# bgmanuel99/Super-Resolution-Images-for-3D-Printing-Defect-Detection

Measured on AMD Instinct MI355X. Metric: 4x-SR MPix/s on 512x512 LR batch, higher is better.
Workload: dtype bf16

## Files before the change

__graft_entry__.py:

```python
import os
import subprocess
import sys

ROOT = os.path.dirname(os.path.abspath(__file__))
PKG = os.path.join(ROOT, "super-resolution-images-for-3d-printing-defect-detection_amd")
for p in (ROOT, PKG):
    if p not in sys.path:
        sys.path.insert(0, p)


def build():
    jobs = str(min(4, os.cpu_count() or 1))
    subprocess.run(["make", "-C", os.path.join(PKG, "csrc"), "-j", jobs], check=True)
    subprocess.run([sys.executable, os.path.join(ROOT, "tools", "check_prefetch_hazards.py")], check=True)
    import sr355
    from sr355 import _lib
    _lib.load()
    import SRModels.loading_methods
    import oracle


def smoke():
    import numpy as np
    import torch
    assert torch.cuda.is_available(), "smoke() needs a GPU"
    from oracle import models as OM
    from oracle import ops as OO
    from sr355 import Context
    from sr355.synth import make_pairs
    from sr355.weights import bf16_rounded, init_weights
    from SRModels.deep_learning_models.ESRGAN_model import ESRGAN

    ctx = Context.get(0)
    lr, hr = make_pairs(1, 40, 36, 4, seed=7)
    for dtype, tol in (("f32", 1e-4), ("bf16", 2e-2)):
        m = ESRGAN(compute_dtype=dtype)
        m.setup_model(scale_factor=4, growth_channels=32, num_rrdb_blocks=2)
        w = init_weights(m.generator.layer_shapes(), seed=3000)
        if dtype == "bf16":
            w = bf16_rounded(w)
        m.set_weights(w)
        sr, metrics = m.super_resolve_image(lr[0], patch_size_lr=24, stride=12)
        ref = OM.esrgan_super_resolve(lr[0], w, 4, 24, 12, num_rrdb=2, dtype=np.float64)
        err = float(np.abs(sr - ref).max())
        assert sr.shape == (160, 144, 3) and err <= tol, (dtype, err)
        p_gpu = float(ctx.psnr(ctx.to_device(hr), ctx.to_device(sr[None]))[0])
        p_ref = float(OO.psnr(hr, ref[None].astype(np.float32))[0])
        assert abs(p_gpu - p_ref) <= 0.01, (p_gpu, p_ref)
        print(f"smoke[{dtype}]: max|gpu-oracle|={err:.2e}  PSNR(gpu,HR)={p_gpu:.4f} dB  PSNR(oracle,HR)={p_ref:.4f} dB  "
              f"time_sec={metrics['time_sec']:.4f}")
    print("smoke OK")


if __name__ == "__main__":
    build()
    if len(sys.argv) > 1 and sys.argv[1] == "smoke":
        smoke()
```

super-resolution-images-for-3d-printing-defect-detection_amd/csrc/attention.hip:

```cpp
#include "attn_f32.h"
#include "common.h"

#include <cstdlib>

namespace {

struct AttnParams {
    const char* qkv; int64_t cs; int qoff, koff, voff;
    char* o; int64_t o_cs; int o_coff;
    int N;
    const float* knorm;
};

__global__ void __launch_bounds__(256, 2) attn_f32_kernel(AttnParams p) {
    __shared__ __attribute__((aligned(16))) char vt[32 * ATTN_VT_PITCH];
    const int b = blockIdx.y;
    const float* base = reinterpret_cast<const float*>(p.qkv) + (int64_t)b * p.N * p.cs;
    const AttnF32Args a{base + p.qoff, base + p.koff, base + p.voff, p.cs, p.cs, p.cs,
                        reinterpret_cast<float*>(p.o) + (int64_t)b * p.N * p.o_cs + p.o_coff, p.o_cs, nullptr, p.N};
    attn_f32_body<false>(a, blockIdx.x * 128, vt);
}

constexpr int KT2 = 128;
constexpr int PITCH2 = KT2 * 2 + 8;

__global__ void __launch_bounds__(64) attn_knorm_kernel(const bf16_t* qkv, int64_t cs, int koff, int N, int ngroups, float* out) {
    const int g = blockIdx.x % ngroups, b = blockIdx.x / ngroups, lane = threadIdx.x;
    const bf16_t* base = qkv + (int64_t)b * N * cs + koff;
    float m = 0.f;
#pragma unroll
    for (int t = 0; t < 2; ++t) {
        const int key = g * 128 + t * 64 + lane;
        if (key < N) {
            const bf16x8 k = *reinterpret_cast<const bf16x8*>(base + (int64_t)key * cs);
            float n2 = 0.f;
#pragma unroll
            for (int e = 0; e < 8; ++e) n2 += (float)k[e] * (float)k[e];
            m = fmaxf(m, n2);
        }
    }
#pragma unroll
    for (int o = 32; o > 0; o >>= 1) m = fmaxf(m, __shfl_xor(m, o));
    if (lane == 0) out[(int64_t)b * ngroups + g] = sqrtf(m);
}

template <int QB>
__global__ void __launch_bounds__(256, 3) attn_bf16_kernel(AttnParams p) {
    __shared__ __attribute__((aligned(16))) char vt[32 * PITCH2];
    const int tid = threadIdx.x, lane = tid & 63, wave = tid >> 6, r = lane & 31, h = lane >> 5;
    const int N = p.N;
    constexpr int QW = 64 * QB * 2;
    const int nqt = (N + QW - 1) / QW;
    const int b = blockIdx.x / nqt, qt = blockIdx.x - b * nqt;
    const bf16_t* base = reinterpret_cast<const bf16_t*>(p.qkv) + (int64_t)b * N * p.cs;
    const int cs = (int)p.cs;
    int qi[QB];
    bf16x8 qb[QB];
#pragma unroll
    for (int j = 0; j < QB; ++j) {
        qi[j] = qt * QW + wave * (32 * QB) + j * 32 + r;
        const int qc = qi[j] < N ? qi[j] : N - 1;
        bf16x8 z = {};
        qb[j] = z;
        if (h == 0) qb[j] = *reinterpret_cast<const bf16x8*>(base + (int64_t)qc * cs + p.qoff);
    }
    float qn2 = 0.f;
#pragma unroll
    for (int j = 0; j < QB; ++j) {
        float n2 = 0.f;
#pragma unroll
        for (int e = 0; e < 8; ++e) n2 += (float)qb[j][e] * (float)qb[j][e];
        qn2 = fmaxf(qn2, n2);
    }
#pragma unroll
    for (int o = 32; o > 0; o >>= 1) qn2 = fmaxf(qn2, __shfl_xor(qn2, o));
    const float qmaxv = sqrtf(qn2) * 1.0009765625f;
    const int* knorm_bits = reinterpret_cast<const int*>(p.knorm) + (int64_t)b * ((N + KT2 - 1) / KT2);
    f32x16 oacc[QB];
    bf16x8 sel = {};
    {
        const int m = lane & 15, kg = lane >> 4;
        const bf16_t one = (bf16_t)1.f;
        if ((m == 0 && (kg & 1) == 0) || (m == 1 && (kg & 1) == 1)) sel = bf16x8{one, one, one, one, one, one, one, one};
    }
    f32x4 lacc[QB];
    float m_run[QB];
#pragma unroll
    for (int j = 0; j < QB; ++j) {
        m_run[j] = 0.f; lacc[j] = f32x4{0.f, 0.f, 0.f, 0.f};
#pragma unroll
        for (int e = 0; e < 16; ++e) oacc[j][e] = 0.f;
    }

    const int kp = tid >> 2, oct = tid & 3;
    bf16x8 kneg = {};
    kneg[0] = (bf16_t)-1.f; kneg[1] = (bf16_t)-1.f; kneg[2] = (bf16_t)-1.f;
    auto load_k = [&](int kb) {
        int l;
        asm volatile("v_mbcnt_lo_u32_b32 %0, -1, 0\n\tv_mbcnt_hi_u32_b32 %0, -1, %0" : "=v"(l));
        bf16x8 kf = kneg;
        const int key = kb + (l & 31);
        if (l < 32) kf = *reinterpret_cast<const bf16x8*>(base + (int64_t)(key < N ? key : N - 1) * cs + p.koff);
        return kf;
    };
    bf16x8 knext = load_k(0);
    f32x16 zero16;
#pragma unroll
    for (int e = 0; e < 16; ++e) zero16[e] = 0.f;
    struct { } false_c; struct { int x; } true_c{0};
    auto hmax = [](float v) {
        const unsigned u = __builtin_bit_cast(unsigned, v);
        const auto sw = __builtin_amdgcn_permlane32_swap(u, u, false, false);
        return fmaxf(__builtin_bit_cast(float, (unsigned)sw[0]), __builtin_bit_cast(float, (unsigned)sw[1]));
    };
    auto tile = [&](const bf16x8 kf, const int sub, const int kb, auto ragged_tag, const bool first) {
        constexpr bool RAGGED = sizeof(ragged_tag) > 1;
        f32x16 s[QB];
        float mx[QB];
#pragma unroll
        for (int j = 0; j < QB; ++j) {
            s[j] = __builtin_amdgcn_mfma_f32_32x32x16_bf16(kf, qb[j], zero16, 0, 0, 0);
            if constexpr (RAGGED) {
#pragma unroll
                for (int i = 0; i < 16; ++i)
                    if (kb + (i & 3) + 8 * (i >> 2) + 4 * h >= N) s[j][i] = -INFINITY;
            }
            float m = fmaxf(fmaxf(s[j][0], s[j][1]), s[j][2]);
#pragma unroll
            for (int i = 3; i + 1 < 16; i += 2) m = fmaxf(fmaxf(m, s[j][i]), s[j][i + 1]);
            m = fmaxf(m, s[j][15]);
            mx[j] = hmax(m);
        }
        bool grew = first;
#pragma unroll
        for (int j = 0; j < QB; ++j) grew = grew || mx[j] > 0.f;
        if (__any(grew)) {
#pragma unroll
            for (int j = 0; j < QB; ++j) {
                const float delta = first ? mx[j] : fmaxf(mx[j], 0.f);
                const float alpha = first ? 1.f : __builtin_amdgcn_exp2f(-delta);
                lacc[j][0] *= alpha;
                lacc[j][1] *= __shfl(alpha, (lane + 16) & 63);
#pragma unroll
                for (int e = 0; e < 16; ++e) oacc[j][e] *= alpha;
#pragma unroll
                for (int i = 0; i < 16; ++i) s[j][i] -= delta;
                m_run[j] += delta;
                if (h == 1) {
                    const bf16_t m1 = (bf16_t)m_run[j];
                    const float r1 = m_run[j] - (float)m1;
                    const bf16_t m2 = (bf16_t)r1;
                    qb[j][0] = m1; qb[j][1] = m2; qb[j][2] = (bf16_t)(r1 - (float)m2);
                }
            }
        }
#pragma unroll
        for (int j = 0; j < QB; ++j) {
#pragma unroll
            for (int i = 0; i < 16; ++i) s[j][i] = __builtin_amdgcn_exp2f(s[j][i]);
        }
#pragma unroll
        for (int ks = 0; ks < 2; ++ks) {
            const char* vrow = vt + r * PITCH2 + (sub * 32 + 16 * ks + 4 * h) * 2;
            const bf16x4 va = *reinterpret_cast<const bf16x4*>(vrow);
            const bf16x4 vb = *reinterpret_cast<const bf16x4*>(vrow + 16);
            const bf16x8 vf = {va[0], va[1], va[2], va[3], vb[0], vb[1], vb[2], vb[3]};
#pragma unroll
            for (int j = 0; j < QB; ++j) {
                bf16x8 pf;
#pragma unroll
                for (int e = 0; e < 8; ++e) pf[e] = (bf16_t)s[j][8 * ks + e];
                oacc[j] = __builtin_amdgcn_mfma_f32_32x32x16_bf16(vf, pf, oacc[j], 0, 0, 0);
                lacc[j] = __builtin_amdgcn_mfma_f32_16x16x32_bf16(sel, pf, lacc[j], 0, 0, 0);
            }
        }
    };

    constexpr float GROW_OK = 40.f;
    auto tile_fast = [&](const bf16x8 kf, const int sub, const bool guard) -> bool {
        f32x16 s[QB];
#pragma unroll
        for (int j = 0; j < QB; ++j) s[j] = __builtin_amdgcn_mfma_f32_32x32x16_bf16(kf, qb[j], zero16, 0, 0, 0);
        if (guard) {
            bool risky = false;
#pragma unroll
            for (int j = 0; j < QB; ++j) {
                float m = fmaxf(fmaxf(s[j][0], s[j][1]), s[j][2]);
#pragma unroll
                for (int i = 3; i + 1 < 16; i += 2) m = fmaxf(fmaxf(m, s[j][i]), s[j][i + 1]);
                m = fmaxf(m, s[j][15]);
                risky = risky || m > GROW_OK;
            }
            if (__any(risky)) return false;
        }
#pragma unroll
        for (int j = 0; j < QB; ++j) {
#pragma unroll
            for (int i = 0; i < 16; ++i) s[j][i] = __builtin_amdgcn_exp2f(s[j][i]);
        }
#pragma unroll
        for (int ks = 0; ks < 2; ++ks) {
            const char* vrow = vt + r * PITCH2 + (sub * 32 + 16 * ks + 4 * h) * 2;
            const bf16x4 va = *reinterpret_cast<const bf16x4*>(vrow);
            const bf16x4 vb = *reinterpret_cast<const bf16x4*>(vrow + 16);
            const bf16x8 vf = {va[0], va[1], va[2], va[3], vb[0], vb[1], vb[2], vb[3]};
#pragma unroll
            for (int j = 0; j < QB; ++j) {
                bf16x8 pf;
#pragma unroll
                for (int e = 0; e < 8; ++e) pf[e] = (bf16_t)s[j][8 * ks + e];
                oacc[j] = __builtin_amdgcn_mfma_f32_32x32x16_bf16(vf, pf, oacc[j], 0, 0, 0);
                lacc[j] = __builtin_amdgcn_mfma_f32_16x16x32_bf16(sel, pf, lacc[j], 0, 0, 0);
            }
        }
        return true;
    };
    auto thresh_of_wave = [&]() -> int {
        float m = m_run[0];
#pragma unroll
        for (int j = 1; j < QB; ++j) m = fminf(m, m_run[j]);
#pragma unroll
        for (int o = 32; o > 0; o >>= 1) m = fminf(m, __shfl_xor(m, o));
        const float lim = GROW_OK + m;
        const float th = !(lim >= 0.f) ? -1.f : (qmaxv > 0.f ? lim / qmaxv * 0.9990234375f : INFINITY);
        return __builtin_amdgcn_readfirstlane(__builtin_bit_cast(int, th));
    };
    int thresh_bits = __builtin_amdgcn_readfirstlane(__builtin_bit_cast(int, -1.f));
    auto stage_v = [&](const int k0) {
        __syncthreads();
#pragma unroll
        for (int part = 0; part < KT2 / 128; ++part) {
            const int ka = k0 + part * 128 + 2 * kp, kbb = ka + 1;
            if (ka - 2 * kp >= N) break;
            const bf16x8 va = *reinterpret_cast<const bf16x8*>(base + (int64_t)(ka < N ? ka : N - 1) * cs + p.voff + oct * 8);
            const bf16x8 vb = *reinterpret_cast<const bf16x8*>(base + (int64_t)(kbb < N ? kbb : N - 1) * cs + p.voff + oct * 8);
#pragma unroll
            for (int e = 0; e < 8; ++e) {
                typedef bf16_t bf16x2 __attribute__((ext_vector_type(2)));
                bf16x2 pr = {va[e], vb[e]};
                *reinterpret_cast<bf16x2*>(vt + (oct * 8 + e) * PITCH2 + (part * 64 + kp) * 4) = pr;
            }
        }
        __syncthreads();
    };
    auto slow_tiles = [&](const int k0, const int sub0, bf16x8 kf) {
        for (int sub = sub0; sub < KT2 / 32; ++sub) {
            const int kb = k0 + sub * 32;
            if (kb >= N) break;
            if (sub != sub0) { kf = knext; knext = load_k(kb + 32); }
            if (kb + 32 <= N) tile(kf, sub, kb, false_c, kb == 0);
            else tile(kf, sub, kb, true_c, kb == 0);
        }
    };

    for (int k0 = 0; k0 < N; k0 += KT2) {
        stage_v(k0);
        int sub = 0;
        bf16x8 kf = knext;
        const bool full = k0 != 0 && k0 + KT2 <= N;
        if (full) {
            const bool guard = !(knorm_bits[k0 / KT2] <= thresh_bits);
#pragma unroll
            for (; sub < KT2 / 32; ++sub) {
                kf = knext;
                knext = load_k(k0 + sub * 32 + 32);
                if (!tile_fast(kf, sub, guard)) break;
            }
        } else {
            knext = load_k(k0 + 32);
        }
        if (sub < KT2 / 32) {
            slow_tiles(k0, sub, kf);
            thresh_bits = thresh_of_wave();
        }
    }
#pragma unroll
    for (int j = 0; j < QB; ++j) {
        const float l0 = __shfl(lacc[j][0], r & 15), l1 = __shfl(lacc[j][1], r & 15);
        const float inv = 1.f / ((r >> 4) ? l1 : l0);
        if (qi[j] < N) {
            bf16_t* op = reinterpret_cast<bf16_t*>(p.o) + ((int64_t)b * N + qi[j]) * p.o_cs + p.o_coff;
#pragma unroll
            for (int g = 0; g < 4; ++g) {
                bf16x4 t = {(bf16_t)(oacc[j][4 * g] * inv), (bf16_t)(oacc[j][4 * g + 1] * inv), (bf16_t)(oacc[j][4 * g + 2] * inv),
                            (bf16_t)(oacc[j][4 * g + 3] * inv)};
                *reinterpret_cast<bf16x4*>(op + 8 * g + 4 * h) = t;
            }
        }
    }
}

}

int attention_launch(sr_ctx* ctx, int dtype, const void* qkv, int64_t cs, int qoff, int koff, int voff, int B, int N,
                     void* o, int64_t o_cs, int o_coff, hipStream_t st) {
    if (B <= 0 || N <= 0) return ctx->fail(SR_ERR_INVALID, "attention: empty tensor");
    const int esz = dtype_size(dtype);
    if ((cs * esz) % 16 || (qoff * esz) % 16 || (koff * esz) % 16 || (voff * esz) % 16 || (o_cs * esz) % 16 || (o_coff * esz) % 16)
        return ctx->fail(SR_ERR_INVALID, "attention: views must be 16-byte aligned");
    AttnParams p{static_cast<const char*>(qkv), cs, qoff, koff, voff, static_cast<char*>(o), o_cs, o_coff, N, nullptr};
    dim3 grid((unsigned)((N + 127) / 128), (unsigned)B);
    if (dtype != SR_DTYPE_BF16 && dtype != SR_DTYPE_F32) return ctx->fail(SR_ERR_INVALID, "attention: dtype must be f32 or bf16");
    const int rec = ctx->prof_open(dtype == SR_DTYPE_BF16 ? "attn<bf16>" : "attn<f32>", 2.0 * B * (double)N * N * 40.0,
                                   (double)B * N * 80.0 * esz, st);
    if (dtype == SR_DTYPE_BF16) {
        constexpr int QBr = 2;
        const int64_t nwg = (int64_t)B * ((N + 128 * QBr - 1) / (128 * QBr));
        const int ngroups = (N + KT2 - 1) / KT2;
        if (nwg >= (1ll << 31) || (int64_t)B * ngroups >= (1ll << 31)) { ctx->prof_close(rec, st); return ctx->fail(SR_ERR_INVALID, "attention: too many workgroups for one launch"); }
        float* kn = static_cast<float*>(ctx->arena(ctx->attn_kn, sizeof(float) * (size_t)B * ngroups, st));
        if (!kn) { ctx->prof_close(rec, st); return SR_ERR_OOM; }
        p.knorm = kn;
        hipLaunchKernelGGL(attn_knorm_kernel, dim3((unsigned)((int64_t)B * ngroups)), dim3(64), 0, st, reinterpret_cast<const bf16_t*>(qkv) + 0, cs, koff, N, ngroups, kn);
        hipLaunchKernelGGL(attn_bf16_kernel<QBr>, dim3((unsigned)nwg), dim3(256), 0, st, p);
    }
    else hipLaunchKernelGGL(attn_f32_kernel, grid, dim3(256), 0, st, p);
    ctx->prof_close(rec, st);
    SR_HIP(ctx, hipGetLastError());
    return SR_OK;
}
```

Before: 110.4.

## Add batched fast path for consecutive skippable-free attention key tiles with asm prefetch

Adds a fast loop in the bf16 attention kernel that uses a wave ballot over precomputed key norms to find a run of consecutive KV blocks where the unguarded fast tile path is safe. Those blocks are then processed without bounds checks or per-tile guards, using inline-asm double-buffered K loads that issue the next tile's global load while the current tile's MFMAs run. The change also specializes V staging for whole tiles to drop clamping. It relies on hand-written waitcnt and exec manipulation, which is why a prefetch hazard checker is added to the build. It also risks register-allocation and correctness issues.

```diff
diff --git a/__graft_entry__.py b/__graft_entry__.py
--- a/__graft_entry__.py
+++ b/__graft_entry__.py
@@ -13,6 +13,8 @@
     jobs = str(min(4, os.cpu_count() or 1))
     subprocess.run(["make", "-C", os.path.join(PKG, "csrc"), "-j", jobs], check=True)
     subprocess.run([sys.executable, os.path.join(ROOT, "tools", "check_prefetch_hazards.py")], check=True)
+    subprocess.run([sys.executable, os.path.join(ROOT, "tools", "check_prefetch_hazards.py"), "--source", os.path.join(PKG, "csrc", "attention.hip"),
+                    "--match", "attn_bf16_kernel", "--allow-scratch"], check=True)
     import sr355
     from sr355 import _lib
     _lib.load()
diff --git a/super-resolution-images-for-3d-printing-defect-detection_amd/csrc/attention.hip b/super-resolution-images-for-3d-printing-defect-detection_amd/csrc/attention.hip
--- a/super-resolution-images-for-3d-printing-defect-detection_amd/csrc/attention.hip
+++ b/super-resolution-images-for-3d-printing-defect-detection_amd/csrc/attention.hip
@@ -226,14 +226,15 @@
         return __builtin_amdgcn_readfirstlane(__builtin_bit_cast(int, th));
     };
     int thresh_bits = __builtin_amdgcn_readfirstlane(__builtin_bit_cast(int, -1.f));
-    auto stage_v = [&](const int k0) {
+    auto stage_v = [&](const int k0, auto whole_tag) {
+        constexpr bool WHOLE = sizeof(whole_tag) > 1;
         __syncthreads();
 #pragma unroll
         for (int part = 0; part < KT2 / 128; ++part) {
             const int ka = k0 + part * 128 + 2 * kp, kbb = ka + 1;
-            if (ka - 2 * kp >= N) break;
-            const bf16x8 va = *reinterpret_cast<const bf16x8*>(base + (int64_t)(ka < N ? ka : N - 1) * cs + p.voff + oct * 8);
-            const bf16x8 vb = *reinterpret_cast<const bf16x8*>(base + (int64_t)(kbb < N ? kbb : N - 1) * cs + p.voff + oct * 8);
+            if (!WHOLE && ka - 2 * kp >= N) break;
+            const bf16x8 va = *reinterpret_cast<const bf16x8*>(base + (int64_t)(WHOLE || ka < N ? ka : N - 1) * cs + p.voff + oct * 8);
+            const bf16x8 vb = *reinterpret_cast<const bf16x8*>(base + (int64_t)(WHOLE || kbb < N ? kbb : N - 1) * cs + p.voff + oct * 8);
 #pragma unroll
             for (int e = 0; e < 8; ++e) {
                 typedef bf16_t bf16x2 __attribute__((ext_vector_type(2)));
@@ -253,25 +254,65 @@
         }
     };
 
-    for (int k0 = 0; k0 < N; k0 += KT2) {
-        stage_v(k0);
-        int sub = 0;
-        bf16x8 kf = knext;
-        const bool full = k0 != 0 && k0 + KT2 <= N;
-        if (full) {
-            const bool guard = !(knorm_bits[k0 / KT2] <= thresh_bits);
-#pragma unroll
-            for (; sub < KT2 / 32; ++sub) {
-                kf = knext;
-                knext = load_k(k0 + sub * 32 + 32);
-                if (!tile_fast(kf, sub, guard)) break;
-            }
-        } else {
-            knext = load_k(k0 + 32);
-        }
-        if (sub < KT2 / 32) {
-            slow_tiles(k0, sub, kf);
-            thresh_bits = thresh_of_wave();
+    const unsigned kvoff = (unsigned)r * (unsigned)cs * 2u;
+    auto fetch_k = [&](bf16x8& use, bf16x8& next, const char* tile_base) {
+        asm volatile("s_waitcnt vmcnt(0)\n\ts_mov_b32 exec_hi, 0\n\tglobal_load_dwordx4 %1, %2, %3\n\ts_mov_b32 exec_hi, -1"
+                     : "+v"(use), "+v"(next) : "v"(kvoff), "s"(tile_base) : "memory");
+    };
+    const int nfast = N % KT2 == 0 ? N / KT2 : (N - 32) / KT2;
+    auto fast_run = [&](const int g) -> int {
+        if (g >= nfast) return 0;
+        int l;
+        asm volatile("v_mbcnt_lo_u32_b32 %0, -1, 0\n\tv_mbcnt_hi_u32_b32 %0, -1, %0" : "=v"(l));
+        const int gi = g + l;
+        const bool ok = gi < nfast && knorm_bits[gi < nfast ? gi : nfast - 1] <= thresh_bits;
+        const unsigned long long fails = ~__ballot(ok);
+        return fails ? __builtin_ctzll(fails) : 64;
+    };
+    const char* const kimg = reinterpret_cast<const char*>(base + p.koff);
+    const int64_t tile_bytes = (int64_t)32 * cs * 2;
+
+    for (int k0 = 0; k0 < N;) {
+        {
+            stage_v(k0, false_c);
+            int sub = 0;
+            bf16x8 kf = knext;
+            const bool full = k0 != 0 && k0 + KT2 <= N;
+            if (full) {
+                const bool guard = !(knorm_bits[k0 / KT2] <= thresh_bits);
+#pragma unroll
+                for (; sub < KT2 / 32; ++sub) {
+                    kf = knext;
+                    knext = load_k(k0 + sub * 32 + 32);
+                    if (!tile_fast(kf, sub, guard)) break;
+                }
+            } else {
+                knext = load_k(k0 + 32);
+            }
+            if (sub < KT2 / 32) {
+                slow_tiles(k0, sub, kf);
+                thresh_bits = thresh_of_wave();
+            }
+            k0 += KT2;
+        }
+        int run = fast_run(k0 / KT2);
+        if (run > 0) {
+            bf16x8 ka = knext, kb = kneg;
+            const char* kt = kimg + (int64_t)(k0 + 32) * cs * 2;
+            do {
+                stage_v(k0, true_c);
+                fetch_k(ka, kb, kt); kt += tile_bytes;
+                tile_fast(ka, 0, false);
+                fetch_k(kb, ka, kt); kt += tile_bytes;
+                tile_fast(kb, 1, false);
+                fetch_k(ka, kb, kt); kt += tile_bytes;
+                tile_fast(ka, 2, false);
+                fetch_k(kb, ka, k0 + KT2 + 32 <= N ? kt : kt - tile_bytes); kt += tile_bytes;
+                tile_fast(kb, 3, false);
+                k0 += KT2;
+            } while (--run);
+            asm volatile("s_waitcnt vmcnt(0)" : "+v"(ka));
+            knext = ka;
         }
     }
 #pragma unroll
```

Result: faster. 112.8 (median of 6 runs) (+2.2%).
